# openai/Video-Pre-Training

Measured on NVIDIA H100. Metric: frames/sec MinecraftPolicy fwd, 128x128x3 BxT=128x128, higher is better.
Workload: dtype bf16

## Files before the change

video-pre-training_b200/csrc/common.cuh:

```cuda
#pragma once
#include <cuda.h>
#include <cuda_bf16.h>
#include <cuda_runtime.h>
#include <stdint.h>

#include "../../include/vpt_b200.h"

namespace vpt {

void set_error(const char* fmt, ...);
#define VPT_CHECK(cond, ...)                 \
    do {                                     \
        if (!(cond)) {                       \
            vpt::set_error(__VA_ARGS__);     \
            return VPT_ERR_ARG;              \
        }                                    \
    } while (0)
#define VPT_CUDA(expr)                                                                   \
    do {                                                                                 \
        cudaError_t _e = (expr);                                                         \
        if (_e != cudaSuccess) {                                                         \
            vpt::set_error("%s failed: %s (%s:%d)", #expr, cudaGetErrorString(_e), __FILE__, __LINE__); \
            return VPT_ERR_CUDA;                                                         \
        }                                                                                \
// ... 33 lines not shown
    for (int o = 16; o > 0; o >>= 1) v += __shfl_xor_sync(0xffffffffu, v, o);
    return v;
}
__device__ __forceinline__ float warp_max(float v) {
#pragma unroll
    for (int o = 16; o > 0; o >>= 1) v = fmaxf(v, __shfl_xor_sync(0xffffffffu, v, o));
    return v;
}

__device__ __forceinline__ uint32_t pack_bf16(float lo, float hi) {
    __nv_bfloat162 v = __floats2bfloat162_rn(lo, hi);
    return *reinterpret_cast<uint32_t*>(&v);
}
__device__ __forceinline__ float bf16_lo(uint32_t v) { return __uint_as_float(v << 16); }
__device__ __forceinline__ float bf16_hi(uint32_t v) { return __uint_as_float(v & 0xffff0000u); }
__device__ __forceinline__ float round_bf16(float v) { return __bfloat162float(__float2bfloat16_rn(v)); }

__device__ __forceinline__ void mbar_init(uint64_t* bar, uint32_t count) {
    asm volatile("mbarrier.init.shared::cta.b64 [%0], %1;" ::"r"(smem_u32(bar)), "r"(count));
}
__device__ __forceinline__ void fence_barrier_init() { asm volatile("fence.mbarrier_init.release.cluster;" ::: "memory"); }
__device__ __forceinline__ void fence_proxy_async() { asm volatile("fence.proxy.async.shared::cta;" ::: "memory"); }
__device__ __forceinline__ void mbar_expect_tx(uint64_t* bar, uint32_t bytes) {
    asm volatile("mbarrier.arrive.expect_tx.shared::cta.b64 _, [%0], %1;" ::"r"(smem_u32(bar)), "r"(bytes) : "memory");
}
__device__ __forceinline__ void mbar_arrive(uint64_t* bar) {
    asm volatile("mbarrier.arrive.shared::cta.b64 _, [%0];" ::"r"(smem_u32(bar)) : "memory");
}
__device__ __forceinline__ bool mbar_try_wait(uint64_t* bar, uint32_t parity) {
    uint32_t ok;
    asm volatile(
        "{\n\t.reg .pred p;\n\t"
        "mbarrier.try_wait.parity.shared::cta.b64 p, [%1], %2;\n\t"
        "selp.b32 %0, 1, 0, p;\n\t}"
        : "=r"(ok)
        : "r"(smem_u32(bar)), "r"(parity)
        : "memory");
    return ok != 0;
}
__device__ __forceinline__ bool mbar_try_wait_sleep(uint64_t* bar, uint32_t parity, uint32_t ns) {
    uint32_t ok;
    asm volatile(
        "{\n\t.reg .pred p;\n\t"
        "mbarrier.try_wait.parity.shared::cta.b64 p, [%1], %2, %3;\n\t"
        "selp.b32 %0, 1, 0, p;\n\t}"
        : "=r"(ok)
        : "r"(smem_u32(bar)), "r"(parity), "r"(ns)
        : "memory");
    return ok != 0;
}
__device__ __forceinline__ bool mbar_wait(uint64_t* bar, uint32_t parity, unsigned int code) {
    if (mbar_try_wait(bar, parity)) return true;
    const long long t0 = clock64();
    for (unsigned int it = 1;; ++it) {
        if (mbar_try_wait_sleep(bar, parity, 20000u)) return true;
        if ((it & 63u) == 0u) {
            if (*(volatile unsigned int*)&g_device_error != 0u) return false;
            if (clock64() - t0 > 3000000000LL) {
                atomicCAS(&g_device_error, 0u, code);
                return false;
            }
        }
    }
}

__device__ __forceinline__ void tma_prefetch_desc(const CUtensorMap* m) {
    asm volatile("prefetch.tensormap [%0];" ::"l"((uint64_t)m) : "memory");
}
__device__ __forceinline__ void tma_load_2d(void* dst, const CUtensorMap* m, uint64_t* bar, int c0, int c1) {
    asm volatile(
        "cp.async.bulk.tensor.2d.shared::cluster.global.tile.mbarrier::complete_tx::bytes [%0], [%1, {%3, %4}], [%2];" ::"r"(
            smem_u32(dst)),
        "l"((uint64_t)m), "r"(smem_u32(bar)), "r"(c0), "r"(c1)
        : "memory");
}
__device__ __forceinline__ void tma_load_4d(void* dst, const CUtensorMap* m, uint64_t* bar, int c0, int c1, int c2, int c3) {
    asm volatile(
        "cp.async.bulk.tensor.4d.shared::cluster.global.tile.mbarrier::complete_tx::bytes [%0], [%1, {%3, %4, %5, %6}], [%2];" ::"r"(
            smem_u32(dst)),
        "l"((uint64_t)m), "r"(smem_u32(bar)), "r"(c0), "r"(c1), "r"(c2), "r"(c3)
        : "memory");
}

__device__ __forceinline__ void tma_store_2d(const CUtensorMap* m, const void* src, int c0, int c1) {
    asm volatile("cp.async.bulk.tensor.2d.global.shared::cta.bulk_group [%0, {%2, %3}], [%1];" ::"l"((uint64_t)m), "r"(smem_u32(src)), "r"(c0),
                 "r"(c1)
                 : "memory");
}
__device__ __forceinline__ void bulk_commit() { asm volatile("cp.async.bulk.commit_group;" ::: "memory"); }
template <int N>
__device__ __forceinline__ void bulk_wait_read() {
    asm volatile("cp.async.bulk.wait_group.read %0;" ::"n"(N) : "memory");
}
template <int N>
__device__ __forceinline__ void bulk_wait_all() {
    asm volatile("cp.async.bulk.wait_group %0;" ::"n"(N) : "memory");
}
__device__ __forceinline__ void named_bar_sync(int id, int nthreads) { asm volatile("bar.sync %0, %1;" ::"r"(id), "r"(nthreads) : "memory"); }
__device__ __forceinline__ void named_bar_arrive(int id, int nthreads) { asm volatile("bar.arrive %0, %1;" ::"r"(id), "r"(nthreads) : "memory"); }

__device__ __forceinline__ void tma_load_2d_mc(void* dst, const CUtensorMap* m, uint64_t* bar, int c0, int c1, uint16_t cta_mask) {
    asm volatile(
        "cp.async.bulk.tensor.2d.shared::cluster.global.tile.mbarrier::complete_tx::bytes.multicast::cluster [%0], [%1, {%3, %4}], [%2], %5;" ::"r"(
            smem_u32(dst)),
        "l"((uint64_t)m), "r"(smem_u32(bar)), "r"(c0), "r"(c1), "h"(cta_mask)
        : "memory");
}

__device__ __forceinline__ void mbar_arrive_cluster(uint64_t* bar, uint32_t rank) {
    asm volatile(
        "{\n\t.reg .b32 ra;\n\t"
        "mapa.shared::cluster.u32 ra, %0, %1;\n\t"
        "mbarrier.arrive.release.cluster.shared::cluster.b64 _, [ra];\n\t}" ::"r"(smem_u32(bar)),
        "r"(rank)
        : "memory");
}
__device__ __forceinline__ uint32_t cluster_ctarank() {
    uint32_t r;
    asm volatile("mov.u32 %0, %%cluster_ctarank;" : "=r"(r));
    return r;
}
__device__ __forceinline__ void cluster_sync_all() {
    asm volatile("barrier.cluster.arrive.release.aligned;\n\tbarrier.cluster.wait.acquire.aligned;" ::: "memory");
}

__device__ __forceinline__ void wgmma_fence() { asm volatile("wgmma.fence.sync.aligned;" ::: "memory"); }
__device__ __forceinline__ void wgmma_commit() { asm volatile("wgmma.commit_group.sync.aligned;" ::: "memory"); }
template <int N>
__device__ __forceinline__ void wgmma_wait() { asm volatile("wgmma.wait_group.sync.aligned %0;" ::"n"(N) : "memory"); }
template <int N>
__device__ __forceinline__ void wgmma_reg_fence(float (&d)[N]) {
#pragma unroll
    for (int i = 0; i < N; ++i) asm volatile("" : "+f"(d[i])::"memory");
}

template <int TA, int TB>
__device__ __forceinline__ void wgmma_n64(float (&d)[32], uint64_t a_desc, uint64_t b_desc, uint32_t accumulate) {
    asm volatile(
        "{\n\t.reg .pred p;\n\t"
        "setp.ne.b32 p, %34, 0;\n\t"
        "wgmma.mma_async.sync.aligned.m64n64k16.f32.bf16.bf16 "
        "{%0, %1, %2, %3, %4, %5, %6, %7, %8, %9, %10, %11, %12, %13, %14, %15, %16, %17, %18, %19, %20, %21, %22, %23, %24, %25, %26, %27, %28, %29, %30, %31}, %32, %33, p, 1, 1, %35, %36;\n\t}"
        : "+f"(d[0]), "+f"(d[1]), "+f"(d[2]), "+f"(d[3]), "+f"(d[4]), "+f"(d[5]), "+f"(d[6]), "+f"(d[7]), "+f"(d[8]), "+f"(d[9]), "+f"(d[10]), "+f"(d[11]), "+f"(d[12]), "+f"(d[13]), "+f"(d[14]), "+f"(d[15]), "+f"(d[16]), "+f"(d[17]), "+f"(d[18]), "+f"(d[19]), "+f"(d[20]), "+f"(d[21]), "+f"(d[22]), "+f"(d[23]), "+f"(d[24]), "+f"(d[25]), "+f"(d[26]), "+f"(d[27]), "+f"(d[28]), "+f"(d[29]), "+f"(d[30]), "+f"(d[31])
        : "l"(a_desc), "l"(b_desc), "r"(accumulate), "n"(TA), "n"(TB)
        : "memory");
}

template <int TA, int TB>
__device__ __forceinline__ void wgmma_n128(float (&d)[64], uint64_t a_desc, uint64_t b_desc, uint32_t accumulate) {
    asm volatile(
        "{\n\t.reg .pred p;\n\t"
        "setp.ne.b32 p, %66, 0;\n\t"
        "wgmma.mma_async.sync.aligned.m64n128k16.f32.bf16.bf16 "
        "{%0, %1, %2, %3, %4, %5, %6, %7, %8, %9, %10, %11, %12, %13, %14, %15, %16, %17, %18, %19, %20, %21, %22, %23, %24, %25, %26, %27, %28, %29, %30, %31, %32, %33, %34, %35, %36, %37, %38, %39, %40, %41, %42, %43, %44, %45, %46, %47, %48, %49, %50, %51, %52, %53, %54, %55, %56, %57, %58, %59, %60, %61, %62, %63}, %64, %65, p, 1, 1, %67, %68;\n\t}"
        : "+f"(d[0]), "+f"(d[1]), "+f"(d[2]), "+f"(d[3]), "+f"(d[4]), "+f"(d[5]), "+f"(d[6]), "+f"(d[7]), "+f"(d[8]), "+f"(d[9]), "+f"(d[10]), "+f"(d[11]), "+f"(d[12]), "+f"(d[13]), "+f"(d[14]), "+f"(d[15]), "+f"(d[16]), "+f"(d[17]), "+f"(d[18]), "+f"(d[19]), "+f"(d[20]), "+f"(d[21]), "+f"(d[22]), "+f"(d[23]), "+f"(d[24]), "+f"(d[25]), "+f"(d[26]), "+f"(d[27]), "+f"(d[28]), "+f"(d[29]), "+f"(d[30]), "+f"(d[31]), "+f"(d[32]), "+f"(d[33]), "+f"(d[34]), "+f"(d[35]), "+f"(d[36]), "+f"(d[37]), "+f"(d[38]), "+f"(d[39]), "+f"(d[40]), "+f"(d[41]), "+f"(d[42]), "+f"(d[43]), "+f"(d[44]), "+f"(d[45]), "+f"(d[46]), "+f"(d[47]), "+f"(d[48]), "+f"(d[49]), "+f"(d[50]), "+f"(d[51]), "+f"(d[52]), "+f"(d[53]), "+f"(d[54]), "+f"(d[55]), "+f"(d[56]), "+f"(d[57]), "+f"(d[58]), "+f"(d[59]), "+f"(d[60]), "+f"(d[61]), "+f"(d[62]), "+f"(d[63])
        : "l"(a_desc), "l"(b_desc), "r"(accumulate), "n"(TA), "n"(TB)
        : "memory");
}

template <int R>
__device__ __forceinline__ void setmaxnreg_dec() { asm volatile("setmaxnreg.dec.sync.aligned.u32 %0;" ::"n"(R)); }
template <int R>
__device__ __forceinline__ void setmaxnreg_inc() { asm volatile("setmaxnreg.inc.sync.aligned.u32 %0;" ::"n"(R)); }

__device__ __forceinline__ uint64_t gmma_desc_sw128(uint32_t smem_addr, uint32_t lbo_bytes = 16u, uint32_t sbo_bytes = 1024u) {
    uint64_t d = 0;
// ... 27 lines not shown
```

video-pre-training_b200/csrc/conv_zp.cuh:

```cuda
#pragma once
#include "common.cuh"
#include "gemm_tc.cuh"

namespace vpt {

static int g_cz_dbg = 0;

constexpr int kCzThreads = 384;
constexpr int kCzMaxBStages = 8;
constexpr int kCzProducerRegs = 24, kCzMmaRegs = 240;

constexpr int kCzBarOrder = 1, kCzBarStg = 3, kCzBarWg = 5;

struct ConvZpParams {
    long long Q;
    int H, W, Wp, FS;
    int N, block_n, num_n_tiles, cin, cin_blocks;
    int a_box_rows, a_boxes, a_stage_bytes, b_stages;
    int dbg;
    int bo;
    long long num_m_tiles;
    const float* mr;
    const float* S1;
    const float* S2;
    int relu;
    const __nv_bfloat16* residual;
    __nv_bfloat16* out;
    float* stat_part;
    const float* Ef;
    const float* res_scale;
    const float* res_shift;
};

template <int BN>
__device__ __forceinline__ void cz_mma_k16(float (&acc)[BN / 2], uint64_t a_desc, uint64_t b_desc, uint32_t accumulate) {
    if constexpr (BN == 128)
        wgmma_n128<0, 0>(acc, a_desc, b_desc, accumulate);
    else
        wgmma_n64<0, 0>(acc, a_desc, b_desc, accumulate);
}

template <int BN>
__global__ void __launch_bounds__(kCzThreads, 1)
conv3x3_zp_kernel(const __grid_constant__ CUtensorMap tmA, const __grid_constant__ CUtensorMap tmB, const ConvZpParams p) {
    static_assert(BN == 64 || BN == 128, "BN is 64 or 128");
    pdl_sync();
    extern __shared__ uint8_t smem_raw[];
    const uint32_t raw = smem_u32(smem_raw);
    uint8_t* smem = smem_raw + (((raw + 1023u) & ~1023u) - raw);
    constexpr uint32_t b_stage_bytes = (uint32_t)BN * kBlockK * 2;
    uint8_t* smem_a = smem;
    uint8_t* smem_b = smem + 2 * (size_t)p.a_stage_bytes;
    float* stg = reinterpret_cast<float*>(smem_b + (size_t)p.b_stages * b_stage_bytes);
    uint64_t* bars = reinterpret_cast<uint64_t*>(reinterpret_cast<uint8_t*>(stg) + kStgBytes);
    uint64_t* a_full = bars;
    uint64_t* a_empty = bars + 2;
    uint64_t* b_full = bars + 4;
    uint64_t* b_empty = bars + 4 + kCzMaxBStages;

    const int warp = threadIdx.x >> 5;
    const int lane = threadIdx.x & 31;

    if (warp == 8 && lane == 0) {
        tma_prefetch_desc(&tmA);
        tma_prefetch_desc(&tmB);
        for (int i = 0; i < 2; ++i) {
            mbar_init(&a_full[i], 1);
            mbar_init(&a_empty[i], 1);
        }
        for (int i = 0; i < p.b_stages; ++i) {
            mbar_init(&b_full[i], 1);
            mbar_init(&b_empty[i], 1);
        }
        fence_barrier_init();
    }
    __syncthreads();

    const int num_tiles = (int)(p.num_m_tiles * p.num_n_tiles);
    const int tile_begin = (int)blockIdx.x;
    const int tile_step = (int)gridDim.x;
    const int halo = p.Wp + 1;

    if (warp >= 8) {
        setmaxnreg_dec<kCzProducerRegs>();
        if (warp == 8 && lane == 0) {
            int stage = 0;
            uint32_t phase = 0;
            bool ok = true;
            for (int tile = tile_begin; tile < num_tiles && ok; tile += tile_step) {
                const int m_tile = tile / p.num_n_tiles;
                const int span0 = m_tile * kBlockM - halo;
                for (int cb = 0; cb < p.cin_blocks; ++cb) {
                    if (!(ok = mbar_wait(&a_empty[stage], phase ^ 1u, 0x110u))) break;
                    mbar_expect_tx(&a_full[stage], (uint32_t)p.a_stage_bytes);
                    uint8_t* sa = smem_a + (size_t)stage * p.a_stage_bytes;
                    for (int b = 0; b < p.a_boxes; ++b)
                        tma_load_2d(sa + (size_t)b * p.a_box_rows * 128, &tmA, &a_full[stage], cb * kBlockK, span0 + b * p.a_box_rows);
                    advance(stage, phase, 2);
                }
            }
        } else if (warp == 9 && lane == 0) {
            int stage = 0;
            uint32_t phase = 0;
            bool ok = true;
            for (int tile = tile_begin; tile < num_tiles && ok; tile += tile_step) {
                const int n0 = (tile % p.num_n_tiles) * BN;
                for (int cb = 0; cb < p.cin_blocks && ok; ++cb) {
                    for (int tap = 0; tap < 9; ++tap) {
                        if (!(ok = mbar_wait(&b_empty[stage], phase ^ 1u, 0x120u))) break;
                        mbar_expect_tx(&b_full[stage], b_stage_bytes);
                        tma_load_2d(smem_b + (size_t)stage * b_stage_bytes, &tmB, &b_full[stage], tap * p.cin + cb * kBlockK, n0);
                        advance(stage, phase, p.b_stages);
                    }
                }
            }
        }
        return;
    }

    setmaxnreg_inc<kCzMmaRegs>();
    const int wg = warp >> 2;
    const int wwarp = warp & 3;
    float* my_row = stg + (size_t)(wwarp * 32 + lane) * kStgPitch;
    const int nchunks = BN >> 5;
    const int c_half = (nchunks + 1) >> 1;
    const int P = p.num_n_tiles * 2;
    const bool res_vec = (((uintptr_t)p.residual | (uintptr_t)p.res_scale | (uintptr_t)p.res_shift) & 15) == 0;
    const int b_per_tile = 9 * p.cin_blocks;
    for (int s = wg; tile_begin + s * tile_step < num_tiles; s += 2) {
        const int tile = tile_begin + s * tile_step;
        const bool has_next = tile + tile_step < num_tiles;
        const int m_tile = tile / p.num_n_tiles;
        const int n_tile = tile % p.num_n_tiles;
        const int n0 = n_tile * BN;
        const long long a_it = (long long)s * p.cin_blocks, b_it = (long long)s * b_per_tile;
        int astage = (int)(a_it & 1), bstage = (int)(b_it % p.b_stages);
        uint32_t aphase = (uint32_t)((a_it >> 1) & 1), bphase = (uint32_t)((b_it / p.b_stages) & 1);

        if (s > 0) named_bar_sync(kCzBarOrder + wg, 256);
        float frag[2][BN / 2];
        bool ok = true;
        int prev_b = -1, prev_a = -1;
        for (int cb = 0; cb < p.cin_blocks && ok; ++cb) {
            if (!(ok = mbar_wait(&a_full[astage], aphase, 0x310u))) break;
            const uint32_t a_base = smem_u32(smem_a + (size_t)astage * p.a_stage_bytes);
#pragma unroll 1
            for (int tap = 0; tap < 9; ++tap) {
                if (!(ok = mbar_wait(&b_full[bstage], bphase, 0x320u))) break;
                const uint32_t b_addr = smem_u32(smem_b + (size_t)bstage * b_stage_bytes);
                const int row_off = (tap / 3) * p.Wp + (tap % 3);
                const uint32_t a_addr = a_base + (uint32_t)row_off * 128u;
                const uint64_t a_bo = p.bo ? ((uint64_t)((a_addr >> 7) & 7u) << 49) : 0ull;
                wgmma_fence();
#pragma unroll
                for (int k = 0; k < kBlockK / 16; ++k) {
                    const uint32_t acc = (uint32_t)((cb | tap | k) != 0);
                    const uint64_t bd = gmma_desc_sw128(b_addr + k * 32);
                    cz_mma_k16<BN>(frag[0], gmma_desc_sw128(a_addr + k * 32) | a_bo, bd, acc);
                    cz_mma_k16<BN>(frag[1], gmma_desc_sw128(a_addr + 64u * 128u + k * 32) | a_bo, bd, acc);
                }
                wgmma_commit();
                wgmma_wait<1>();
                if ((threadIdx.x & 127) == 0) {
                    if (prev_b >= 0) mbar_arrive(&b_empty[prev_b]);
                    if (prev_a >= 0) mbar_arrive(&a_empty[prev_a]);
                }
                prev_a = -1;
                prev_b = bstage;
                advance(bstage, bphase, p.b_stages);
            }
            prev_a = astage;
            advance(astage, aphase, 2);
        }
        if (has_next) named_bar_arrive(kCzBarOrder + (wg ^ 1), 256);
        wgmma_wait<0>();
#pragma unroll
        for (int h = 0; h < 2; ++h) wgmma_reg_fence(frag[h]);
        if ((threadIdx.x & 127) == 0) {
            if (prev_b >= 0) mbar_arrive(&b_empty[prev_b]);
            if (prev_a >= 0) mbar_arrive(&a_empty[prev_a]);
        }
        if (!ok) {
            if (has_next) named_bar_arrive(kCzBarStg + (wg ^ 1), 256);
            break;
        }

        if (s > 0) named_bar_sync(kCzBarStg + wg, 256);
#pragma unroll
        for (int h = 0; h < 2; ++h) wgmma_frag_store(frag[h], stg + (size_t)h * 64 * kStgPitch, kStgPitch, 0);
        named_bar_sync(kCzBarWg + wg, 128);

        const int q = m_tile * kBlockM + wwarp * 32 + lane;
        const bool row_ok = q < p.Q;
        const int f = q / p.FS;
        const int r = q - f * p.FS;
        const int y = r / p.Wp, x = r - y * p.Wp;
        const bool interior = row_ok && (y < p.H) && (x < p.W);
        float ga = 1.f, gb = 0.f;
        if (p.mr != nullptr && interior) {
            const float mean = __ldg(p.mr + 2 * f), rstd = __ldg(p.mr + 2 * f + 1);
            ga = rstd;
            gb = rstd * mean;
        }
        const int cy = (y == 0) ? 0 : ((y == p.H - 1) ? 2 : 1);
        const int cx = (x == 0) ? 0 : ((x == p.W - 1) ? 2 : 1);
        const int cls = interior ? cy * 3 + cx : 0;
        const float* s1row = p.S1 ? p.S1 + (size_t)cls * p.N : nullptr;
        const float* s2row = p.S2 ? p.S2 + (size_t)cls * p.N : nullptr;
        if (p.Ef) {
            s1row = nullptr;
            s2row = p.Ef + ((size_t)(interior ? f : 0) * 9 + cls) * p.N;
        }
        const float* rarow = (p.res_scale && interior) ? p.res_scale + (size_t)f * p.N : nullptr;
        const float* rbrow = (p.res_scale && interior) ? p.res_shift + (size_t)f * p.N : nullptr;
        float st_s0 = 0.f, st_ss0 = 0.f, st_s1 = 0.f, st_ss1 = 0.f;

        const int qw = m_tile * kBlockM + wwarp * 32;
        float* wrows = stg + (size_t)(wwarp * 32) * kStgPitch;
        const int seg = lane & 3;
#pragma unroll 1
        for (int c = 0; c < (p.dbg == 2 ? 0 : nchunks); ++c) {
            const int g = c < c_half ? 0 : 1;
            const int nb = n0 + c * 32;
            const int lim = min(32, min(BN - c * 32, p.N - nb));
            if (lim <= 0) break;
            const bool full = (lim == 32) && ((p.N & 7) == 0) && res_vec;
            uint32_t acc[32];
            float v[32];
            uint32_t pk[16];
            if (full) {
                stg_ld_32(my_row + c * 32, acc);
                __syncwarp();
                if (p.residual != nullptr) {
#pragma unroll
                    for (int k = 0; k < 4; ++k) {
                        const int rr = 8 * k + (lane >> 2);
                        if (qw + rr < p.Q)
                            reinterpret_cast<uint4*>(wrows + (size_t)rr * kStgPitch + c * 32)[seg] =
                                __ldg(reinterpret_cast<const uint4*>(p.residual + (size_t)(qw + rr) * p.N + nb) + seg);
                    }
                    __syncwarp();
                }
                if (row_ok) {
                    if (!interior) {
#pragma unroll
                        for (int j = 0; j < 16; ++j) pk[j] = 0u;
                    } else {
#pragma unroll
                        for (int qq = 0; qq < 8; ++qq) {
                            float4 a1 = s1row ? __ldg(reinterpret_cast<const float4*>(s1row + nb) + qq) : make_float4(0, 0, 0, 0);
                            float4 a2 = s2row ? __ldg(reinterpret_cast<const float4*>(s2row + nb) + qq) : make_float4(0, 0, 0, 0);
                            v[4 * qq + 0] = fmaf(ga, __uint_as_float(acc[4 * qq + 0]), fmaf(-gb, a1.x, a2.x));
                            v[4 * qq + 1] = fmaf(ga, __uint_as_float(acc[4 * qq + 1]), fmaf(-gb, a1.y, a2.y));
                            v[4 * qq + 2] = fmaf(ga, __uint_as_float(acc[4 * qq + 2]), fmaf(-gb, a1.z, a2.z));
                            v[4 * qq + 3] = fmaf(ga, __uint_as_float(acc[4 * qq + 3]), fmaf(-gb, a1.w, a2.w));
                        }
                        if (p.relu == 1) {
#pragma unroll
                            for (int j = 0; j < 32; ++j) v[j] = fmaxf(v[j], 0.f);
                        }
                        if (p.residual != nullptr) {
                            const uint4* rp = reinterpret_cast<const uint4*>(my_row + c * 32);
#pragma unroll
                            for (int qq = 0; qq < 4; ++qq) {
                                const uint4 rr = rp[qq];
                                const float r8[8] = {bf16_lo(rr.x), bf16_hi(rr.x), bf16_lo(rr.y), bf16_hi(rr.y),
                                                     bf16_lo(rr.z), bf16_hi(rr.z), bf16_lo(rr.w), bf16_hi(rr.w)};
                                if (rarow) {
                                    const float4* ra4 = reinterpret_cast<const float4*>(rarow + nb) + 2 * qq;
                                    const float4* rb4 = reinterpret_cast<const float4*>(rbrow + nb) + 2 * qq;
                                    const float4 a0 = __ldg(ra4), a1 = __ldg(ra4 + 1), b0 = __ldg(rb4), b1 = __ldg(rb4 + 1);
                                    const float ra[8] = {a0.x, a0.y, a0.z, a0.w, a1.x, a1.y, a1.z, a1.w};
                                    const float rb[8] = {b0.x, b0.y, b0.z, b0.w, b1.x, b1.y, b1.z, b1.w};
#pragma unroll
                                    for (int j = 0; j < 8; ++j) v[8 * qq + j] += fmaf(ra[j], r8[j], rb[j]);
                                } else {
#pragma unroll
                                    for (int j = 0; j < 8; ++j) v[8 * qq + j] += r8[j];
                                }
                            }
                        }
                        if (p.relu == 2) {
#pragma unroll
                            for (int j = 0; j < 32; ++j) v[j] = fmaxf(v[j], 0.f);
                        }
#pragma unroll
                        for (int j = 0; j < 16; ++j) pk[j] = pack_bf16(v[2 * j], v[2 * j + 1]);
                        if (p.stat_part) {
                            float s_ = g ? st_s1 : st_s0, ss_ = g ? st_ss1 : st_ss0;
#pragma unroll
                            for (int j = 0; j < 16; ++j) {
                                const float lo = bf16_lo(pk[j]), hi = bf16_hi(pk[j]);
                                s_ += lo; ss_ = fmaf(lo, lo, ss_);
                                s_ += hi; ss_ = fmaf(hi, hi, ss_);
                            }
                            if (g) { st_s1 = s_; st_ss1 = ss_; } else { st_s0 = s_; st_ss0 = ss_; }
                        }
                    }
#pragma unroll
                    for (int qq = 0; qq < 4; ++qq)
                        reinterpret_cast<uint4*>(my_row + c * 32 + 16)[qq] = make_uint4(pk[4 * qq], pk[4 * qq + 1], pk[4 * qq + 2], pk[4 * qq + 3]);
                }
                __syncwarp();
                if (p.dbg != 1) {
#pragma unroll
                    for (int k = 0; k < 4; ++k) {
                        const int rr = 8 * k + (lane >> 2);
                        if (qw + rr < p.Q)
                            reinterpret_cast<uint4*>(p.out + (size_t)(qw + rr) * p.N + nb)[seg] =
                                reinterpret_cast<const uint4*>(wrows + (size_t)rr * kStgPitch + c * 32 + 16)[seg];
                    }
                }
                continue;
            }
            if (!row_ok) continue;
            stg_ld_32(my_row + c * 32, acc);
            __nv_bfloat16* op = p.out + (size_t)q * p.N + nb;
            if (!interior) {
                for (int j = 0; j < lim; ++j) op[j] = __float2bfloat16_rn(0.f);
                continue;
            }
#pragma unroll
            for (int j = 0; j < 32; ++j) {
                float a1 = 0.f, a2 = 0.f;
                if (j < lim) {
                    if (s1row) a1 = __ldg(s1row + nb + j);
                    if (s2row) a2 = __ldg(s2row + nb + j);
                }
                v[j] = fmaf(ga, __uint_as_float(acc[j]), fmaf(-gb, a1, a2));
            }
            if (p.relu == 1) {
#pragma unroll
                for (int j = 0; j < 32; ++j) v[j] = fmaxf(v[j], 0.f);
            }
            if (p.residual != nullptr) {
                const __nv_bfloat16* rp = p.residual + (size_t)q * p.N + nb;
#pragma unroll
                for (int j = 0; j < 32; ++j)
                    if (j < lim) v[j] += rarow ? fmaf(__ldg(rarow + nb + j), __bfloat162float(rp[j]), __ldg(rbrow + nb + j)) : __bfloat162float(rp[j]);
            }
            if (p.relu == 2) {
#pragma unroll
                for (int j = 0; j < 32; ++j) v[j] = fmaxf(v[j], 0.f);
            }
#pragma unroll
            for (int j = 0; j < 16; ++j) pk[j] = pack_bf16(v[2 * j], v[2 * j + 1]);
            if (p.stat_part) {
                float s_ = g ? st_s1 : st_s0, ss_ = g ? st_ss1 : st_ss0;
#pragma unroll
                for (int j = 0; j < 16; ++j) {
                    const float lo = bf16_lo(pk[j]), hi = bf16_hi(pk[j]);
                    if (2 * j < lim) { s_ += lo; ss_ = fmaf(lo, lo, ss_); }
                    if (2 * j + 1 < lim) { s_ += hi; ss_ = fmaf(hi, hi, ss_); }
                }
                if (g) { st_s1 = s_; st_ss1 = ss_; } else { st_s0 = s_; st_ss0 = ss_; }
            }
            if (p.dbg != 1) {
#pragma unroll
                for (int j = 0; j < 32; ++j)
                    if (j < lim) op[j] = __float2bfloat16_rn(v[j]);
            }
        }
        if (has_next) named_bar_arrive(kCzBarStg + (wg ^ 1), 256);
        if (p.stat_part && row_ok)
            reinterpret_cast<float4*>(p.stat_part)[((size_t)q * P + n_tile * 2) >> 1] = make_float4(st_s0, st_ss0, st_s1, st_ss1);
    }
}

}

namespace vpt {
static inline void conv_zp_block_n(long long Q, int N, int* bn, int* nt) {
    choose_block_n(N, bn, nt);
    const long long tiles = (Q + kBlockM - 1) / kBlockM;
    if (tiles * *nt >= 64 || *bn == 64) return;
    *bn = 64;
    *nt = (N + 63) / 64;
}
}

extern "C" int vpt_conv3x3_zp(const vpt_conv_zp_args* a, void* stream) {
    using namespace vpt;
    VPT_CHECK(a && a->x && a->w && a->out, "vpt_conv3x3_zp: null operand");
    const int H = a->H, W = a->W, C = a->Cin, N = a->Cout;
    VPT_CHECK(a->F > 0 && H >= 2 && W >= 2 && C > 0 && C % 64 == 0 && N > 0 && N % 16 == 0,
              "vpt_conv3x3_zp: need F>0, H,W>=2, Cin %% 64 == 0, Cout %% 16 == 0 (F=%d H=%d W=%d Cin=%d Cout=%d)", a->F, H, W, C, N);
    VPT_CHECK(W <= 182, "vpt_conv3x3_zp: W=%d too wide (at most 182: two input spans of 128 + 2*(W+2) rows must fit in shared memory)", W);
    VPT_CHECK(((uintptr_t)a->x & 15) == 0 && ((uintptr_t)a->w & 15) == 0 && ((uintptr_t)a->out & 15) == 0, "vpt_conv3x3_zp: pointers must be 16-byte aligned");
    ConvZpParams p;
    memset(&p, 0, sizeof(p));
    p.H = H; p.W = W; p.Wp = W + 1; p.FS = (H + 1) * (W + 1);
    p.Q = (long long)a->F * p.FS;
    VPT_CHECK(p.Q <= 2147483647LL - kBlockM, "vpt_conv3x3_zp: too many rows for 32-bit row indices and TMA coordinates");
    p.N = N; p.cin = C; p.cin_blocks = C / 64;
    conv_zp_block_n(p.Q, N, &p.block_n, &p.num_n_tiles);
    p.num_m_tiles = (p.Q + kBlockM - 1) / kBlockM;
    const int span = kBlockM + 2 * (p.Wp + 1);
    p.a_boxes = (span + 255) / 256;
    p.a_box_rows = ((span + p.a_boxes - 1) / p.a_boxes + 7) / 8 * 8;
    VPT_CHECK(p.a_box_rows <= 256, "vpt_conv3x3_zp: span does not fit the TMA box limit");
    p.a_stage_bytes = p.a_boxes * p.a_box_rows * 128;
    const uint32_t b_stage_bytes = (uint32_t)p.block_n * kBlockK * 2;
    const size_t fixed_bytes = 1024 + 2 * (size_t)p.a_stage_bytes + kStgBytes + (4 + 2 * kCzMaxBStages) * 8;
    int bst = (int)((227 * 1024 - (long long)fixed_bytes) / b_stage_bytes);
    if (bst > kCzMaxBStages) bst = kCzMaxBStages;
    VPT_CHECK(bst >= 2, "vpt_conv3x3_zp: not enough shared memory for the weight pipeline (W=%d Cout=%d)", W, N);
    p.b_stages = bst;
    const size_t smem_bytes = fixed_bytes + (size_t)bst * b_stage_bytes;

    CUtensorMap tmA, tmB;
    {
        cuuint64_t dims[2] = {(cuuint64_t)C, (cuuint64_t)p.Q};
        cuuint64_t strides[1] = {(cuuint64_t)C * 2};
        cuuint32_t box[2] = {64, (cuuint32_t)p.a_box_rows};
        int r = make_tmap_bf16(&tmA, a->x, 2, dims, strides, box);
        if (r) return r;
    }
    {
        cuuint64_t dims[2] = {(cuuint64_t)9 * C, (cuuint64_t)N};
        cuuint64_t strides[1] = {(cuuint64_t)9 * C * 2};
        cuuint32_t box[2] = {64, (cuuint32_t)p.block_n};
        int r = make_tmap_bf16(&tmB, a->w, 2, dims, strides, box);
        if (r) return r;
    }
    VPT_CHECK(!(a->mr && !a->S1 && !a->Ef), "vpt_conv3x3_zp: mr given without S1 (or Ef)");
    VPT_CHECK(!a->Ef || a->mr, "vpt_conv3x3_zp: Ef needs mr = (0, rstd) per frame");
    VPT_CHECK(!a->res_scale == !a->res_shift && (!a->res_scale || a->residual) && (!a->res_scale || N % 8 == 0),
              "vpt_conv3x3_zp: res_scale / res_shift come as a pair, with a residual, Cout %% 8 == 0");
    p.mr = a->mr; p.S1 = a->mr ? a->S1 : nullptr; p.S2 = a->S2; p.relu = a->relu;
    p.residual = reinterpret_cast<const __nv_bfloat16*>(a->residual);
    p.out = reinterpret_cast<__nv_bfloat16*>(a->out);
    p.stat_part = a->stat_part;
    p.Ef = a->Ef; p.res_scale = a->res_scale; p.res_shift = a->res_shift;
    p.dbg = g_cz_dbg;
    p.bo = g_dbg_bo > 0 ? 1 : 0;

    static bool attr_set = false;
    if (!attr_set) {
        VPT_CUDA(cudaFuncSetAttribute(conv3x3_zp_kernel<64>, cudaFuncAttributeMaxDynamicSharedMemorySize, 227 * 1024));
        VPT_CUDA(cudaFuncSetAttribute(conv3x3_zp_kernel<128>, cudaFuncAttributeMaxDynamicSharedMemorySize, 227 * 1024));
        attr_set = true;
    }
    const long long tiles = p.num_m_tiles * p.num_n_tiles;
    long long grid = num_sms();
    if (grid <= 0) grid = 132;
    if (grid > tiles) grid = tiles;
    if (p.block_n == 64)
        launch_k(conv3x3_zp_kernel<64>, dim3((unsigned)grid), dim3(kCzThreads), smem_bytes, (cudaStream_t)stream, tmA, tmB, p);
    else
        launch_k(conv3x3_zp_kernel<128>, dim3((unsigned)grid), dim3(kCzThreads), smem_bytes, (cudaStream_t)stream, tmA, tmB, p);
    VPT_LAUNCH_CHECK();
    return VPT_OK;
}

extern "C" int vpt_set_conv_pair_mode(int32_t on) {
    vpt::g_cz_dbg = (on & 0xff) >> 4;
    return VPT_OK;
}

extern "C" int vpt_set_conv_swap_mode(int32_t on) {
    (void)on;
    return VPT_OK;
}

extern "C" int64_t vpt_conv_zp_t_stat_floats(int32_t F, int32_t H, int32_t W, int32_t Cout) {
    (void)F; (void)H; (void)W; (void)Cout;
    return 0;
}

extern "C" int vpt_conv_zp_t_stats_finalize(const float* part, float* mr, int32_t F, int32_t H, int32_t W, float eps, void* stream) {
    (void)part; (void)mr; (void)F; (void)H; (void)W; (void)eps; (void)stream;
    vpt::set_error("vpt_conv_zp_t_stats_finalize: no convolution kernel of this build emits per-tile partials (vpt_conv_zp_t_stat_floats is 0)");
    return VPT_ERR_ARG;
}

extern "C" int vpt_conv_zp_stat_parts(int32_t F, int32_t H, int32_t W, int32_t Cout) {
    const long long Q = (long long)F * (H + 1) * (W + 1);
    int bn, nt;
    vpt::conv_zp_block_n(Q, Cout, &bn, &nt);
    return nt * 2;
}
```

Measured before the change: 20530.

## Rewrite conv epilogue to stage tiles in swizzled smem with TMA residual/output

After: 21740, median of 6. +5.9%, better.

```diff
diff --git a/video-pre-training_b200/csrc/common.cuh b/video-pre-training_b200/csrc/common.cuh
--- a/video-pre-training_b200/csrc/common.cuh
+++ b/video-pre-training_b200/csrc/common.cuh
@@ -139,6 +139,12 @@
         : "memory");
 }
 
+__device__ __forceinline__ void bulk_load(void* dst, const void* src, uint32_t bytes, uint64_t* bar) {
+    asm volatile("cp.async.bulk.shared::cluster.global.mbarrier::complete_tx::bytes [%0], [%1], %2, [%3];" ::"r"(smem_u32(dst)),
+                 "l"((uint64_t)src), "r"(bytes), "r"(smem_u32(bar))
+                 : "memory");
+}
+
 __device__ __forceinline__ void tma_store_2d(const CUtensorMap* m, const void* src, int c0, int c1) {
     asm volatile("cp.async.bulk.tensor.2d.global.shared::cta.bulk_group [%0, {%2, %3}], [%1];" ::"l"((uint64_t)m), "r"(smem_u32(src)), "r"(c0),
                  "r"(c1)
diff --git a/video-pre-training_b200/csrc/conv_zp.cuh b/video-pre-training_b200/csrc/conv_zp.cuh
--- a/video-pre-training_b200/csrc/conv_zp.cuh
+++ b/video-pre-training_b200/csrc/conv_zp.cuh
@@ -10,7 +10,10 @@
 constexpr int kCzMaxBStages = 8;
 constexpr int kCzProducerRegs = 24, kCzMmaRegs = 240;
 
-constexpr int kCzBarOrder = 1, kCzBarStg = 3, kCzBarWg = 5;
+constexpr int kCzBarOrder = 1, kCzBarWg = 3;
+constexpr uint32_t kCzBoxBytes = (uint32_t)kBlockM * 128u;
+constexpr int kCzBarBytes = 256;
+constexpr int kCzTabMinStages = 4;
 
 struct ConvZpParams {
     long long Q;
@@ -30,6 +33,8 @@
     const float* Ef;
     const float* res_scale;
     const float* res_shift;
+    int tab_mask, tab_bytes;
+    int tab_off[5];
 };
 
 template <int BN>
@@ -40,23 +45,139 @@
         wgmma_n64<0, 0>(acc, a_desc, b_desc, accumulate);
 }
 
-template <int BN>
+__host__ __device__ __forceinline__ long long cz_tab_size(const ConvZpParams& p, int t) {
+    const long long F = p.Q / p.FS;
+    return 4LL * p.N * (t < 2 ? 9 : (t == 2 ? 9 * F : F));
+}
+
+__device__ const float g_cz_zero[kMaxBlockN] = {};
+
+struct CzTables {
+    const float* S1;
+    const float* S2;
+    const float* Ef;
+    const float* ra;
+    const float* rb;
+};
+__device__ __forceinline__ CzTables cz_tables(const ConvZpParams& p, const uint8_t* tabs) {
+    auto pick = [&](int t, const float* g) { return (p.tab_mask >> t) & 1 ? reinterpret_cast<const float*>(tabs + p.tab_off[t]) : g; };
+    return CzTables{pick(0, p.S1), pick(1, p.S2), pick(2, p.Ef), pick(3, p.res_scale), pick(4, p.res_shift)};
+}
+
+struct CzRow {
+    bool interior, affine;
+    float ga, gb;
+    const float* s1;
+    const float* s2;
+    const float* ra;
+    const float* rb;
+};
+__device__ __forceinline__ CzRow cz_row(const ConvZpParams& p, const CzTables& t, int q, int n0) {
+    CzRow w;
+    const int f = q / p.FS;
+    const int r = q - f * p.FS;
+    const int y = r / p.Wp, x = r - y * p.Wp;
+    w.interior = q < p.Q && (y < p.H) && (x < p.W);
+    w.ga = 1.f;
+    w.gb = 0.f;
+    if (p.mr != nullptr && w.interior) {
+        const float mean = __ldg(p.mr + 2 * f), rstd = __ldg(p.mr + 2 * f + 1);
+        w.ga = rstd;
+        w.gb = rstd * mean;
+    }
+    const int cy = (y == 0) ? 0 : ((y == p.H - 1) ? 2 : 1);
+    const int cx = (x == 0) ? 0 : ((x == p.W - 1) ? 2 : 1);
+    const int cls = w.interior ? cy * 3 + cx : 0;
+    w.s1 = p.S1 ? t.S1 + (size_t)cls * p.N + n0 : g_cz_zero;
+    w.s2 = p.S2 ? t.S2 + (size_t)cls * p.N + n0 : g_cz_zero;
+    if (p.Ef) {
+        w.s1 = g_cz_zero;
+        w.s2 = t.Ef + ((size_t)(w.interior ? f : 0) * 9 + cls) * p.N + n0;
+    }
+    w.affine = p.res_scale && w.interior;
+    w.ra = w.affine ? t.ra + (size_t)f * p.N + n0 : g_cz_zero;
+    w.rb = w.affine ? t.rb + (size_t)f * p.N + n0 : g_cz_zero;
+    return w;
+}
+
+__device__ __forceinline__ void cz_stat8(const uint4 u, float& s, float& ss) {
+    const uint32_t w[4] = {u.x, u.y, u.z, u.w};
+#pragma unroll
+    for (int j = 0; j < 4; ++j) {
+        const float lo = bf16_lo(w[j]), hi = bf16_hi(w[j]);
+        s += lo; ss = fmaf(lo, lo, ss);
+        s += hi; ss = fmaf(hi, hi, ss);
+    }
+}
+
+template <int BN, bool RES, bool AFFINE>
+__device__ __forceinline__ void cz_epilogue_frag(const ConvZpParams& p, float (&frag)[2][BN / 2], uint8_t* tb, const uint8_t* tabs, int qt,
+                                                 int n0, int wwarp, int lane) {
+    const int l4 = lane >> 2;
+    const CzTables t = cz_tables(p, tabs);
+#pragma unroll
+    for (int h = 0; h < 2; ++h) {
+#pragma unroll
+        for (int e = 0; e < 2; ++e) {
+            const int row = 64 * h + 16 * wwarp + 8 * e + l4;
+            const CzRow rw = cz_row(p, t, qt + row, n0);
+            uint8_t* rp = tb + (size_t)row * 128 + 4 * (lane & 3);
+            const int c0 = 2 * (lane & 3);
+#pragma unroll
+            for (int i = 0; i < BN / 8; ++i) {
+                uint32_t* cell = reinterpret_cast<uint32_t*>(rp + (i >> 3) * kCzBoxBytes + (((i & 7) ^ l4) << 4));
+                const bool col_ok = n0 + 8 * i < p.N;
+                const int c = c0 + 8 * i;
+                const float2 a1 = *reinterpret_cast<const float2*>(rw.s1 + (col_ok ? c : c0));
+                const float2 a2 = *reinterpret_cast<const float2*>(rw.s2 + (col_ok ? c : c0));
+                float v0 = fmaf(rw.ga, frag[h][4 * i + 2 * e], fmaf(-rw.gb, a1.x, a2.x));
+                float v1 = fmaf(rw.ga, frag[h][4 * i + 2 * e + 1], fmaf(-rw.gb, a1.y, a2.y));
+                v0 = p.relu == 1 ? fmaxf(v0, 0.f) : v0;
+                v1 = p.relu == 1 ? fmaxf(v1, 0.f) : v1;
+                if constexpr (RES) {
+                    const uint32_t r2 = *cell;
+                    if constexpr (AFFINE) {
+                        const float2 ra = *reinterpret_cast<const float2*>(rw.ra + (col_ok ? c : c0));
+                        const float2 rb = *reinterpret_cast<const float2*>(rw.rb + (col_ok ? c : c0));
+                        v0 += rw.affine ? fmaf(ra.x, bf16_lo(r2), rb.x) : bf16_lo(r2);
+                        v1 += rw.affine ? fmaf(ra.y, bf16_hi(r2), rb.y) : bf16_hi(r2);
+                    } else {
+                        v0 += bf16_lo(r2);
+                        v1 += bf16_hi(r2);
+                    }
+                }
+                v0 = p.relu == 2 ? fmaxf(v0, 0.f) : v0;
+                v1 = p.relu == 2 ? fmaxf(v1, 0.f) : v1;
+                *cell = (rw.interior && col_ok) ? pack_bf16(v0, v1) : 0u;
+            }
+        }
+    }
+}
+
+template <int BN, int RES>
 __global__ void __launch_bounds__(kCzThreads, 1)
-conv3x3_zp_kernel(const __grid_constant__ CUtensorMap tmA, const __grid_constant__ CUtensorMap tmB, const ConvZpParams p) {
+conv3x3_zp_kernel(const __grid_constant__ CUtensorMap tmA, const __grid_constant__ CUtensorMap tmB,
+                  const __grid_constant__ CUtensorMap tmR, const __grid_constant__ CUtensorMap tmO, const ConvZpParams p) {
     static_assert(BN == 64 || BN == 128, "BN is 64 or 128");
+    static_assert(RES >= 0 && RES <= 2, "RES is 0, 1 or 2");
     pdl_sync();
     extern __shared__ uint8_t smem_raw[];
     const uint32_t raw = smem_u32(smem_raw);
     uint8_t* smem = smem_raw + (((raw + 1023u) & ~1023u) - raw);
     constexpr uint32_t b_stage_bytes = (uint32_t)BN * kBlockK * 2;
+    constexpr uint32_t tile_bytes = (uint32_t)(BN / 64) * kCzBoxBytes;
     uint8_t* smem_a = smem;
     uint8_t* smem_b = smem + 2 * (size_t)p.a_stage_bytes;
-    float* stg = reinterpret_cast<float*>(smem_b + (size_t)p.b_stages * b_stage_bytes);
-    uint64_t* bars = reinterpret_cast<uint64_t*>(reinterpret_cast<uint8_t*>(stg) + kStgBytes);
+    uint8_t* tbuf = smem_b + (size_t)p.b_stages * b_stage_bytes;
+    uint64_t* bars = reinterpret_cast<uint64_t*>(tbuf + 2 * tile_bytes);
     uint64_t* a_full = bars;
     uint64_t* a_empty = bars + 2;
     uint64_t* b_full = bars + 4;
     uint64_t* b_empty = bars + 4 + kCzMaxBStages;
+    uint64_t* r_full = bars + 4 + 2 * kCzMaxBStages;
+    uint64_t* r_empty = r_full + 2;
+    uint64_t* tab_full = r_empty + 2;
+    const uint8_t* tabs = reinterpret_cast<uint8_t*>(bars) + kCzBarBytes;
 
     const int warp = threadIdx.x >> 5;
     const int lane = threadIdx.x & 31;
@@ -67,7 +188,10 @@
         for (int i = 0; i < 2; ++i) {
             mbar_init(&a_full[i], 1);
             mbar_init(&a_empty[i], 1);
-        }
+            mbar_init(&r_full[i], 1);
+            mbar_init(&r_empty[i], 128);
+        }
+        mbar_init(tab_full, 1);
         for (int i = 0; i < p.b_stages; ++i) {
             mbar_init(&b_full[i], 1);
             mbar_init(&b_empty[i], 1);
@@ -114,6 +238,28 @@
                     }
                 }
             }
+        } else if (warp == 10 && lane == 0) {
+            if (p.tab_mask) {
+                const float* src[5] = {p.S1, p.S2, p.Ef, p.res_scale, p.res_shift};
+                mbar_expect_tx(tab_full, (uint32_t)p.tab_bytes);
+                for (int t = 0; t < 5; ++t)
+                    if ((p.tab_mask >> t) & 1)
+                        bulk_load(const_cast<uint8_t*>(tabs) + p.tab_off[t], src[t], (uint32_t)cz_tab_size(p, t), tab_full);
+            }
+            if (RES == 0) return;
+            tma_prefetch_desc(&tmR);
+            bool ok = true;
+            for (int s = 0; tile_begin + s * tile_step < num_tiles && ok; ++s) {
+                const int tile = tile_begin + s * tile_step;
+                const int n0 = (tile % p.num_n_tiles) * BN;
+                const int b = s & 1;
+                if (!(ok = mbar_wait(&r_empty[b], ((uint32_t)(s >> 1) & 1u) ^ 1u, 0x130u))) break;
+                const int nbox = min(BN / 64, (p.N - n0 + 63) / 64);
+                mbar_expect_tx(&r_full[b], (uint32_t)nbox * kCzBoxBytes);
+                for (int j = 0; j < nbox; ++j)
+                    tma_load_2d(tbuf + (size_t)b * tile_bytes + (size_t)j * kCzBoxBytes, &tmR, &r_full[b], n0 + 64 * j,
+                                (tile / p.num_n_tiles) * kBlockM);
+            }
         }
         return;
     }
@@ -121,11 +267,8 @@
     setmaxnreg_inc<kCzMmaRegs>();
     const int wg = warp >> 2;
     const int wwarp = warp & 3;
-    float* my_row = stg + (size_t)(wwarp * 32 + lane) * kStgPitch;
-    const int nchunks = BN >> 5;
-    const int c_half = (nchunks + 1) >> 1;
     const int P = p.num_n_tiles * 2;
-    const bool res_vec = (((uintptr_t)p.residual | (uintptr_t)p.res_scale | (uintptr_t)p.res_shift) & 15) == 0;
+    uint8_t* tb = tbuf + (size_t)wg * tile_bytes;
     const int b_per_tile = 9 * p.cin_blocks;
     for (int s = wg; tile_begin + s * tile_step < num_tiles; s += 2) {
         const int tile = tile_begin + s * tile_step;
@@ -180,191 +323,45 @@
             if (prev_b >= 0) mbar_arrive(&b_empty[prev_b]);
             if (prev_a >= 0) mbar_arrive(&a_empty[prev_a]);
         }
-        if (!ok) {
-            if (has_next) named_bar_arrive(kCzBarStg + (wg ^ 1), 256);
-            break;
-        }
-
-        if (s > 0) named_bar_sync(kCzBarStg + wg, 256);
-#pragma unroll
-        for (int h = 0; h < 2; ++h) wgmma_frag_store(frag[h], stg + (size_t)h * 64 * kStgPitch, kStgPitch, 0);
-        named_bar_sync(kCzBarWg + wg, 128);
-
-        const int q = m_tile * kBlockM + wwarp * 32 + lane;
-        const bool row_ok = q < p.Q;
-        const int f = q / p.FS;
-        const int r = q - f * p.FS;
-        const int y = r / p.Wp, x = r - y * p.Wp;
-        const bool interior = row_ok && (y < p.H) && (x < p.W);
-        float ga = 1.f, gb = 0.f;
-        if (p.mr != nullptr && interior) {
-            const float mean = __ldg(p.mr + 2 * f), rstd = __ldg(p.mr + 2 * f + 1);
-            ga = rstd;
-            gb = rstd * mean;
-        }
-        const int cy = (y == 0) ? 0 : ((y == p.H - 1) ? 2 : 1);
-        const int cx = (x == 0) ? 0 : ((x == p.W - 1) ? 2 : 1);
-        const int cls = interior ? cy * 3 + cx : 0;
-        const float* s1row = p.S1 ? p.S1 + (size_t)cls * p.N : nullptr;
-        const float* s2row = p.S2 ? p.S2 + (size_t)cls * p.N : nullptr;
-        if (p.Ef) {
-            s1row = nullptr;
-            s2row = p.Ef + ((size_t)(interior ? f : 0) * 9 + cls) * p.N;
-        }
-        const float* rarow = (p.res_scale && interior) ? p.res_scale + (size_t)f * p.N : nullptr;
-        const float* rbrow = (p.res_scale && interior) ? p.res_shift + (size_t)f * p.N : nullptr;
+        if (!ok) break;
+
+        const int qt = m_tile * kBlockM;
+        const uint32_t use_par = (uint32_t)(s >> 1) & 1u;
+        if (!(RES ? mbar_wait(&r_full[wg], use_par, 0x330u) : mbar_wait(&r_empty[wg], use_par ^ 1u, 0x340u))) break;
+        if (p.tab_mask && !mbar_wait(tab_full, 0, 0x350u)) break;
         float st_s0 = 0.f, st_ss0 = 0.f, st_s1 = 0.f, st_ss1 = 0.f;
-
-        const int qw = m_tile * kBlockM + wwarp * 32;
-        float* wrows = stg + (size_t)(wwarp * 32) * kStgPitch;
-        const int seg = lane & 3;
-#pragma unroll 1
-        for (int c = 0; c < (p.dbg == 2 ? 0 : nchunks); ++c) {
-            const int g = c < c_half ? 0 : 1;
-            const int nb = n0 + c * 32;
-            const int lim = min(32, min(BN - c * 32, p.N - nb));
-            if (lim <= 0) break;
-            const bool full = (lim == 32) && ((p.N & 7) == 0) && res_vec;
-            uint32_t acc[32];
-            float v[32];
-            uint32_t pk[16];
-            if (full) {
-                stg_ld_32(my_row + c * 32, acc);
-                __syncwarp();
-                if (p.residual != nullptr) {
-#pragma unroll
-                    for (int k = 0; k < 4; ++k) {
-                        const int rr = 8 * k + (lane >> 2);
-                        if (qw + rr < p.Q)
-                            reinterpret_cast<uint4*>(wrows + (size_t)rr * kStgPitch + c * 32)[seg] =
-                                __ldg(reinterpret_cast<const uint4*>(p.residual + (size_t)(qw + rr) * p.N + nb) + seg);
+        const int srow = wwarp * 32 + lane;
+        if (p.dbg != 2) {
+            cz_epilogue_frag<BN, RES != 0, RES == 2>(p, frag, tb, tabs, qt, n0, wwarp, lane);
+            fence_proxy_async();
+            named_bar_sync(kCzBarWg + wg, 128);
+            if ((threadIdx.x & 127) == 0 && p.dbg != 1) {
+                for (int j = 0; j < BN / 64 && n0 + 64 * j < p.N; ++j) tma_store_2d(&tmO, tb + (size_t)j * kCzBoxBytes, n0 + 64 * j, qt);
+                bulk_commit();
+            }
+            if (p.stat_part && cz_row(p, cz_tables(p, tabs), qt + srow, n0).interior) {
+                const uint8_t* rp = tb + (size_t)srow * 128;
+                constexpr int G = BN / 16;
+#pragma unroll
+                for (int k = 0; k < G; ++k) {
+                    if (n0 + 8 * k < p.N) {
+                        const uint4 u = *reinterpret_cast<const uint4*>(rp + (k >> 3) * kCzBoxBytes + (((k & 7) ^ (srow & 7)) << 4));
+                        cz_stat8(u, st_s0, st_ss0);
                     }
-                    __syncwarp();
-                }
-                if (row_ok) {
-                    if (!interior) {
-#pragma unroll
-                        for (int j = 0; j < 16; ++j) pk[j] = 0u;
-                    } else {
-#pragma unroll
-                        for (int qq = 0; qq < 8; ++qq) {
-                            float4 a1 = s1row ? __ldg(reinterpret_cast<const float4*>(s1row + nb) + qq) : make_float4(0, 0, 0, 0);
-                            float4 a2 = s2row ? __ldg(reinterpret_cast<const float4*>(s2row + nb) + qq) : make_float4(0, 0, 0, 0);
-                            v[4 * qq + 0] = fmaf(ga, __uint_as_float(acc[4 * qq + 0]), fmaf(-gb, a1.x, a2.x));
-                            v[4 * qq + 1] = fmaf(ga, __uint_as_float(acc[4 * qq + 1]), fmaf(-gb, a1.y, a2.y));
-                            v[4 * qq + 2] = fmaf(ga, __uint_as_float(acc[4 * qq + 2]), fmaf(-gb, a1.z, a2.z));
-                            v[4 * qq + 3] = fmaf(ga, __uint_as_float(acc[4 * qq + 3]), fmaf(-gb, a1.w, a2.w));
-                        }
-                        if (p.relu == 1) {
-#pragma unroll
-                            for (int j = 0; j < 32; ++j) v[j] = fmaxf(v[j], 0.f);
-                        }
-                        if (p.residual != nullptr) {
-                            const uint4* rp = reinterpret_cast<const uint4*>(my_row + c * 32);
-#pragma unroll
-                            for (int qq = 0; qq < 4; ++qq) {
-                                const uint4 rr = rp[qq];
-                                const float r8[8] = {bf16_lo(rr.x), bf16_hi(rr.x), bf16_lo(rr.y), bf16_hi(rr.y),
-                                                     bf16_lo(rr.z), bf16_hi(rr.z), bf16_lo(rr.w), bf16_hi(rr.w)};
-                                if (rarow) {
-                                    const float4* ra4 = reinterpret_cast<const float4*>(rarow + nb) + 2 * qq;
-                                    const float4* rb4 = reinterpret_cast<const float4*>(rbrow + nb) + 2 * qq;
-                                    const float4 a0 = __ldg(ra4), a1 = __ldg(ra4 + 1), b0 = __ldg(rb4), b1 = __ldg(rb4 + 1);
-                                    const float ra[8] = {a0.x, a0.y, a0.z, a0.w, a1.x, a1.y, a1.z, a1.w};
-                                    const float rb[8] = {b0.x, b0.y, b0.z, b0.w, b1.x, b1.y, b1.z, b1.w};
-#pragma unroll
-                                    for (int j = 0; j < 8; ++j) v[8 * qq + j] += fmaf(ra[j], r8[j], rb[j]);
-                                } else {
-#pragma unroll
-                                    for (int j = 0; j < 8; ++j) v[8 * qq + j] += r8[j];
-                                }
-                            }
-                        }
-                        if (p.relu == 2) {
-#pragma unroll
-                            for (int j = 0; j < 32; ++j) v[j] = fmaxf(v[j], 0.f);
-                        }
-#pragma unroll
-                        for (int j = 0; j < 16; ++j) pk[j] = pack_bf16(v[2 * j], v[2 * j + 1]);
-                        if (p.stat_part) {
-                            float s_ = g ? st_s1 : st_s0, ss_ = g ? st_ss1 : st_ss0;
-#pragma unroll
-                            for (int j = 0; j < 16; ++j) {
-                                const float lo = bf16_lo(pk[j]), hi = bf16_hi(pk[j]);
-                                s_ += lo; ss_ = fmaf(lo, lo, ss_);
-                                s_ += hi; ss_ = fmaf(hi, hi, ss_);
-                            }
-                            if (g) { st_s1 = s_; st_ss1 = ss_; } else { st_s0 = s_; st_ss0 = ss_; }
-                        }
-                    }
-#pragma unroll
-                    for (int qq = 0; qq < 4; ++qq)
-                        reinterpret_cast<uint4*>(my_row + c * 32 + 16)[qq] = make_uint4(pk[4 * qq], pk[4 * qq + 1], pk[4 * qq + 2], pk[4 * qq + 3]);
-                }
-                __syncwarp();
-                if (p.dbg != 1) {
-#pragma unroll
-                    for (int k = 0; k < 4; ++k) {
-                        const int rr = 8 * k + (lane >> 2);
-                        if (qw + rr < p.Q)
-                            reinterpret_cast<uint4*>(p.out + (size_t)(qw + rr) * p.N + nb)[seg] =
-                                reinterpret_cast<const uint4*>(wrows + (size_t)rr * kStgPitch + c * 32 + 16)[seg];
+                    if (n0 + 8 * (k + G) < p.N) {
+                        const int k1 = k + G;
+                        const uint4 u = *reinterpret_cast<const uint4*>(rp + (k1 >> 3) * kCzBoxBytes + (((k1 & 7) ^ (srow & 7)) << 4));
+                        cz_stat8(u, st_s1, st_ss1);
                     }
                 }
-                continue;
-            }
-            if (!row_ok) continue;
-            stg_ld_32(my_row + c * 32, acc);
-            __nv_bfloat16* op = p.out + (size_t)q * p.N + nb;
-            if (!interior) {
-                for (int j = 0; j < lim; ++j) op[j] = __float2bfloat16_rn(0.f);
-                continue;
-            }
-#pragma unroll
-            for (int j = 0; j < 32; ++j) {
-                float a1 = 0.f, a2 = 0.f;
-                if (j < lim) {
-                    if (s1row) a1 = __ldg(s1row + nb + j);
-                    if (s2row) a2 = __ldg(s2row + nb + j);
-                }
-                v[j] = fmaf(ga, __uint_as_float(acc[j]), fmaf(-gb, a1, a2));
-            }
-            if (p.relu == 1) {
-#pragma unroll
-                for (int j = 0; j < 32; ++j) v[j] = fmaxf(v[j], 0.f);
-            }
-            if (p.residual != nullptr) {
-                const __nv_bfloat16* rp = p.residual + (size_t)q * p.N + nb;
-#pragma unroll
-                for (int j = 0; j < 32; ++j)
-                    if (j < lim) v[j] += rarow ? fmaf(__ldg(rarow + nb + j), __bfloat162float(rp[j]), __ldg(rbrow + nb + j)) : __bfloat162float(rp[j]);
-            }
-            if (p.relu == 2) {
-#pragma unroll
-                for (int j = 0; j < 32; ++j) v[j] = fmaxf(v[j], 0.f);
-            }
-#pragma unroll
-            for (int j = 0; j < 16; ++j) pk[j] = pack_bf16(v[2 * j], v[2 * j + 1]);
-            if (p.stat_part) {
-                float s_ = g ? st_s1 : st_s0, ss_ = g ? st_ss1 : st_ss0;
-#pragma unroll
-                for (int j = 0; j < 16; ++j) {
-                    const float lo = bf16_lo(pk[j]), hi = bf16_hi(pk[j]);
-                    if (2 * j < lim) { s_ += lo; ss_ = fmaf(lo, lo, ss_); }
-                    if (2 * j + 1 < lim) { s_ += hi; ss_ = fmaf(hi, hi, ss_); }
-                }
-                if (g) { st_s1 = s_; st_ss1 = ss_; } else { st_s0 = s_; st_ss0 = ss_; }
-            }
-            if (p.dbg != 1) {
-#pragma unroll
-                for (int j = 0; j < 32; ++j)
-                    if (j < lim) op[j] = __float2bfloat16_rn(v[j]);
-            }
-        }
-        if (has_next) named_bar_arrive(kCzBarStg + (wg ^ 1), 256);
-        if (p.stat_part && row_ok)
-            reinterpret_cast<float4*>(p.stat_part)[((size_t)q * P + n_tile * 2) >> 1] = make_float4(st_s0, st_ss0, st_s1, st_ss1);
-    }
+            }
+            if ((threadIdx.x & 127) == 0) bulk_wait_read<0>();
+        }
+        mbar_arrive(&r_empty[wg]);
+        if (p.stat_part && qt + srow < p.Q)
+            reinterpret_cast<float4*>(p.stat_part)[((size_t)(qt + srow) * P + n_tile * 2) >> 1] = make_float4(st_s0, st_ss0, st_s1, st_ss1);
+    }
+    if ((threadIdx.x & 127) == 0) bulk_wait_all<0>();
 }
 
 }
@@ -385,8 +382,12 @@
     const int H = a->H, W = a->W, C = a->Cin, N = a->Cout;
     VPT_CHECK(a->F > 0 && H >= 2 && W >= 2 && C > 0 && C % 64 == 0 && N > 0 && N % 16 == 0,
               "vpt_conv3x3_zp: need F>0, H,W>=2, Cin %% 64 == 0, Cout %% 16 == 0 (F=%d H=%d W=%d Cin=%d Cout=%d)", a->F, H, W, C, N);
-    VPT_CHECK(W <= 182, "vpt_conv3x3_zp: W=%d too wide (at most 182: two input spans of 128 + 2*(W+2) rows must fit in shared memory)", W);
+    VPT_CHECK(W <= 190, "vpt_conv3x3_zp: W=%d too wide (at most 190: two input spans of 128 + 2*(W+2) rows, the tile buffers and two "
+              "weight stages must fit in shared memory)", W);
     VPT_CHECK(((uintptr_t)a->x & 15) == 0 && ((uintptr_t)a->w & 15) == 0 && ((uintptr_t)a->out & 15) == 0, "vpt_conv3x3_zp: pointers must be 16-byte aligned");
+    VPT_CHECK(((uintptr_t)a->residual & 15) == 0, "vpt_conv3x3_zp: residual must be 16-byte aligned (it is read by TMA)");
+    VPT_CHECK((((uintptr_t)a->S1 | (uintptr_t)a->S2 | (uintptr_t)a->Ef | (uintptr_t)a->res_scale | (uintptr_t)a->res_shift) & 15) == 0,
+              "vpt_conv3x3_zp: S1, S2, Ef, res_scale and res_shift must be 16-byte aligned (they are copied by bulk copy)");
     ConvZpParams p;
     memset(&p, 0, sizeof(p));
     p.H = H; p.W = W; p.Wp = W + 1; p.FS = (H + 1) * (W + 1);
@@ -401,14 +402,12 @@
     VPT_CHECK(p.a_box_rows <= 256, "vpt_conv3x3_zp: span does not fit the TMA box limit");
     p.a_stage_bytes = p.a_boxes * p.a_box_rows * 128;
     const uint32_t b_stage_bytes = (uint32_t)p.block_n * kBlockK * 2;
-    const size_t fixed_bytes = 1024 + 2 * (size_t)p.a_stage_bytes + kStgBytes + (4 + 2 * kCzMaxBStages) * 8;
+    const size_t fixed_bytes = 1024 + 2 * (size_t)p.a_stage_bytes + 2 * (size_t)(p.block_n / 64) * kCzBoxBytes + kCzBarBytes;
     int bst = (int)((227 * 1024 - (long long)fixed_bytes) / b_stage_bytes);
     if (bst > kCzMaxBStages) bst = kCzMaxBStages;
     VPT_CHECK(bst >= 2, "vpt_conv3x3_zp: not enough shared memory for the weight pipeline (W=%d Cout=%d)", W, N);
-    p.b_stages = bst;
-    const size_t smem_bytes = fixed_bytes + (size_t)bst * b_stage_bytes;
-
-    CUtensorMap tmA, tmB;
+
+    CUtensorMap tmA, tmB, tmR, tmO;
     {
         cuuint64_t dims[2] = {(cuuint64_t)C, (cuuint64_t)p.Q};
         cuuint64_t strides[1] = {(cuuint64_t)C * 2};
@@ -422,6 +421,15 @@
         cuuint32_t box[2] = {64, (cuuint32_t)p.block_n};
         int r = make_tmap_bf16(&tmB, a->w, 2, dims, strides, box);
         if (r) return r;
+    }
+    {
+        cuuint64_t dims[2] = {(cuuint64_t)N, (cuuint64_t)p.Q};
+        cuuint64_t strides[1] = {(cuuint64_t)N * 2};
+        cuuint32_t box[2] = {64, (cuuint32_t)kBlockM};
+        int r = make_tmap_bf16(&tmO, a->out, 2, dims, strides, box);
+        if (r) return r;
+        tmR = tmO;
+        if (a->residual && (r = make_tmap_bf16(&tmR, a->residual, 2, dims, strides, box))) return r;
     }
     VPT_CHECK(!(a->mr && !a->S1 && !a->Ef), "vpt_conv3x3_zp: mr given without S1 (or Ef)");
     VPT_CHECK(!a->Ef || a->mr, "vpt_conv3x3_zp: Ef needs mr = (0, rstd) per frame");
@@ -435,20 +443,46 @@
     p.dbg = g_cz_dbg;
     p.bo = g_dbg_bo > 0 ? 1 : 0;
 
+    long long left = 227 * 1024 - (long long)fixed_bytes - (long long)bst * b_stage_bytes;
+    const int groups[3] = {(p.S1 && !p.Ef ? 1 : 0) | (p.S2 && !p.Ef ? 2 : 0), p.Ef ? 4 : 0, p.res_scale ? 8 | 16 : 0};
+    for (int g = 0; g < 3; ++g) {
+        long long bytes = 0;
+        for (int t = 0; t < 5; ++t)
+            if ((groups[g] >> t) & 1) bytes += cz_tab_size(p, t);
+        if (bytes == 0) continue;
+        if (g == 0 && bytes > left && bst > kCzTabMinStages) {
+            --bst;
+            left += b_stage_bytes;
+        }
+        if (bytes > left) continue;
+        for (int t = 0; t < 5; ++t)
+            if ((groups[g] >> t) & 1) {
+                p.tab_off[t] = p.tab_bytes;
+                p.tab_bytes += (int)cz_tab_size(p, t);
+            }
+        p.tab_mask |= groups[g];
+        left -= bytes;
+    }
+    p.b_stages = bst;
+    const size_t smem_bytes = fixed_bytes + (size_t)bst * b_stage_bytes + (size_t)p.tab_bytes;
+
+    using Kernel = void (*)(const CUtensorMap, const CUtensorMap, const CUtensorMap, const CUtensorMap, const ConvZpParams);
+    static const Kernel kernels[2][3] = {{conv3x3_zp_kernel<64, 0>, conv3x3_zp_kernel<64, 1>, conv3x3_zp_kernel<64, 2>},
+                                         {conv3x3_zp_kernel<128, 0>, conv3x3_zp_kernel<128, 1>, conv3x3_zp_kernel<128, 2>}};
     static bool attr_set = false;
     if (!attr_set) {
-        VPT_CUDA(cudaFuncSetAttribute(conv3x3_zp_kernel<64>, cudaFuncAttributeMaxDynamicSharedMemorySize, 227 * 1024));
-        VPT_CUDA(cudaFuncSetAttribute(conv3x3_zp_kernel<128>, cudaFuncAttributeMaxDynamicSharedMemorySize, 227 * 1024));
+        for (int b = 0; b < 2; ++b)
+            for (int r = 0; r < 3; ++r)
+                VPT_CUDA(cudaFuncSetAttribute(kernels[b][r], cudaFuncAttributeMaxDynamicSharedMemorySize, 227 * 1024));
         attr_set = true;
     }
     const long long tiles = p.num_m_tiles * p.num_n_tiles;
     long long grid = num_sms();
     if (grid <= 0) grid = 132;
     if (grid > tiles) grid = tiles;
-    if (p.block_n == 64)
-        launch_k(conv3x3_zp_kernel<64>, dim3((unsigned)grid), dim3(kCzThreads), smem_bytes, (cudaStream_t)stream, tmA, tmB, p);
-    else
-        launch_k(conv3x3_zp_kernel<128>, dim3((unsigned)grid), dim3(kCzThreads), smem_bytes, (cudaStream_t)stream, tmA, tmB, p);
+    const int res = a->residual == nullptr ? 0 : (a->res_scale == nullptr ? 1 : 2);
+    launch_k(kernels[p.block_n == 64 ? 0 : 1][res], dim3((unsigned)grid), dim3(kCzThreads), smem_bytes, (cudaStream_t)stream, tmA, tmB, tmR,
+             tmO, p);
     VPT_LAUNCH_CHECK();
     return VPT_OK;
 }
```
